# shiyuan0806/SVDFormer_PointSea

Measured on AMD Instinct MI355X. Metric: train-step samples/sec (PCN, B=32, 2048->16384 pts), higher is better.
Workload: dtype bf16; 1 GPU; SVDFormer PCN train step: render + fwd + get_loss + bwd + Adam; global_batch=32, per_gpu_batch=32, points_in=2048, points_out=16384, params=58092521, parallelism=single

## Files before the change

### include/pcops.h

```cpp
#ifndef PCOPS_H_
#define PCOPS_H_

#ifdef __cplusplus
extern "C" {
#endif

typedef struct ihipStream_t *pcops_stream_t;

enum pcops_status {
  PCOPS_OK = 0,
  PCOPS_ERR_INVALID = 1,
  PCOPS_ERR_LAUNCH = 2,
  PCOPS_ERR_WORKSPACE = 3,
  PCOPS_ERR_UNSUPPORTED = 4
};

const char *pcops_status_string(int status);
int pcops_abi_version(void);


unsigned long long pcops_fps_workspace_bytes(int B, int N);
int pcops_furthest_point_sampling(const float *xyz, int B, int N, int M, int *idx, void *workspace,
                                  unsigned long long workspace_bytes, pcops_stream_t stream);
int pcops_furthest_point_sampling_counts(const float *xyz, const int *counts, int B, int N, int M, int *idx,
// ... 200 lines not shown
int pcops_batchnorm_bwd(const void *dy, const void *y, const void *x, int dtype, long long rows, int C,
                        const float *gamma, const float *save_mean, const float *save_invstd, int batch_stats, int act,
                        float slope, void *dx, void *dres, float *dgamma, float *dbeta, void *workspace,
                        unsigned long long workspace_bytes, pcops_stream_t stream);
int pcops_batchnorm_fwd_save(const void *x, int dtype, const void *res, int res_dtype, long long rows, int C,
                             const float *gamma, const float *beta, float *running_mean, float *running_var,
                             float momentum, float eps, int batch_stats, int act, float slope, void *y,
                             float *save_mean, float *save_invstd, float *save_coef, unsigned char *save_mask,
                             void *workspace, unsigned long long workspace_bytes, long long *num_batches_tracked,
                             pcops_stream_t stream);
int pcops_batchnorm_bwd_saved(const void *dy, const float *save_coef, const unsigned char *save_mask, const void *x,
                              int dtype, long long rows, int C, const float *gamma, const float *save_mean,
                              const float *save_invstd, int batch_stats, int act, float slope, void *dx, void *dres,
                              float *dgamma, float *dbeta, void *workspace, unsigned long long workspace_bytes,
                              pcops_stream_t stream);

int pcops_conv3x3_fwd(const void *x, const void *w, int N, int H, int W, int C, void *y, pcops_stream_t stream);
int pcops_conv3x3_fwd_res(const void *x, const void *w, int N, int H, int W, int C, const void *res, void *y,
                          pcops_stream_t stream);
unsigned long long pcops_conv3x3_wgrad_workspace_bytes(int C);
int pcops_conv3x3_wgrad(const void *x, const void *dy, int N, int H, int W, int C, void *dw, int dw_dtype,
                        int dw_ohwi, void *workspace, unsigned long long workspace_bytes, pcops_stream_t stream);

int pcops_conv3x3_c1_fwd(const float *x, const float *w, int N, int H, int W, void *y, pcops_stream_t stream);
unsigned long long pcops_conv3x3_c1_wgrad_workspace_bytes(void);
int pcops_conv3x3_c1_wgrad(const float *x, const void *dy, int N, int H, int W, void *dw, int dw_dtype, void *workspace,
                           unsigned long long workspace_bytes, pcops_stream_t stream);

int pcops_pcsa_forward(const void *x, int x_dtype, const void *gates, int gates_dtype, const float *basis, int patches,
                       int K, int C, void *out, pcops_stream_t stream);
int pcops_pcsa_backward(const void *x, int x_dtype, const void *dout, int dout_dtype, const void *gates,
                        int gates_dtype, const float *basis, int patches, int K, int C, void *dx, void *dgates,
                        pcops_stream_t stream);

// ... 14 lines not shown
```

### svdformer_pointsea_amd/_lib.py

```python
import ctypes
import os
import threading

import torch

_HERE = os.path.dirname(os.path.abspath(__file__))
LIB_PATH = os.environ.get("PCOPS_LIB_PATH") or os.path.join(_HERE, "_lib", "libpcops.so")

_lib = None

P = ctypes.c_void_p
I = ctypes.c_int
F = ctypes.c_float
D = ctypes.c_double
LL = ctypes.c_longlong
ULL = ctypes.c_ulonglong

_SIGS = {
    "pcops_status_string": (ctypes.c_char_p, [I]),
    "pcops_abi_version": (I, []),
    "pcops_fps_workspace_bytes": (ULL, [I, I]),
    "pcops_furthest_point_sampling": (I, [P, I, I, I, P, P, ULL, P]),
    "pcops_furthest_point_sampling_counts": (I, [P, P, I, I, I, P, P, ULL, P]),
    "pcops_gather_points": (I, [P, P, I, I, I, I, P, P]),
# ... 53 lines not shown
    "pcops_layernorm_bwd_ex": (I, [P, I, LL, P, P, P, I, P, I, P, P, P, I, I, P, P, P, P, P, I, P, ULL, P]),
    "pcops_adam_flat": (I, [P, P, P, LL, LL, P, P, P, P, D, P, D, D, D, D, I, P]),
    "pcops_blend_fwd": (I, [P, I, P, P, LL, P, I, P]),
    "pcops_blend_bwd": (I, [P, I, P, I, P, P, LL, P, P, P, P]),
    "pcops_sum_rows": (I, [P, I, LL, P, I, P]),
    "pcops_wgrad_skinny_workspace_bytes": (ULL, [I, I]),
    "pcops_wgrad_skinny": (I, [P, P, LL, I, I, P, I, P, ULL, P]),
    "pcops_colsum_workspace_bytes": (ULL, [LL, I]),
    "pcops_colsum": (I, [P, I, LL, I, P, I, P, ULL, P]),
    "pcops_colsum_ld": (I, [P, I, LL, I, LL, P, I, P, ULL, P]),
    "pcops_batchnorm_workspace_bytes": (ULL, [LL, I]),
    "pcops_batchnorm_fwd": (I, [P, I, P, I, LL, I, P, P, P, P, F, F, I, I, F, P, P, P, P, ULL, P, P]),
    "pcops_batchnorm_bwd": (I, [P, P, P, I, LL, I, P, P, P, I, I, F, P, P, P, P, P, ULL, P]),
    "pcops_batchnorm_fwd_save": (I, [P, I, P, I, LL, I, P, P, P, P, F, F, I, I, F, P, P, P, P, P, P, ULL, P, P]),
    "pcops_batchnorm_bwd_saved": (I, [P, P, P, P, I, LL, I, P, P, P, I, I, F, P, P, P, P, P, ULL, P]),
    "pcops_conv3x3_fwd": (I, [P, P, I, I, I, I, P, P]),
    "pcops_conv3x3_fwd_res": (I, [P, P, I, I, I, I, P, P, P]),
    "pcops_conv3x3_wgrad_workspace_bytes": (ULL, [I]),
    "pcops_conv3x3_wgrad": (I, [P, P, I, I, I, I, P, I, I, P, ULL, P]),
    "pcops_conv3x3_c1_fwd": (I, [P, P, I, I, I, P, P]),
    "pcops_conv3x3_c1_wgrad_workspace_bytes": (ULL, []),
    "pcops_conv3x3_c1_wgrad": (I, [P, P, I, I, I, P, I, P, ULL, P]),
    "pcops_pcsa_forward": (I, [P, I, P, I, P, I, I, I, P, P]),
    "pcops_pcsa_backward": (I, [P, I, P, I, P, I, P, I, I, I, P, P, P]),
    "pcops_points2depth_workspace_bytes": (ULL, [I, I, I, I]),
    "pcops_points2depth": (I, [P, P, P, I, I, I, I, I, P, P, ULL, P]),
    "pcops_points2grid": (I, [P, P, P, P, I, I, I, I, I, P, P]),
    "pcops_grid2image_workspace_bytes": (ULL, [I, I, I]),
    "pcops_grid2image": (I, [P, P, I, I, I, P, P, ULL, P]),
}

# ... 278 lines not shown
```

### svdformer_pointsea_amd/batchnorm.py

```python
import os

import torch
from torch import nn

from ._lib import Workspace, call, lib, ptr, stream_of

_DT = {torch.float32: 0, torch.bfloat16: 1}
ACT_NONE, ACT_RELU, ACT_LEAKY = 0, 1, 2
ENABLED = os.environ.get("PCOPS_BN", "1") != "0"


def _rows_c(x):
    C = x.shape[1]
    return x.numel() // C, C


def _switch(name):
    return os.environ.get(name, "1") != "0"


def _mask_source(act, has_res):
    if act == ACT_NONE:
        return "y"
    if has_res:
        return "bits" if _switch("PCOPS_BN_MASK_BITS") else "y"
    return "coef" if _switch("PCOPS_BN_RECOMPUTE_MASK") else "y"


class _BNAct(torch.autograd.Function):
    @staticmethod
    def forward(ctx, x, res, weight, bias, rmean, rvar, nbt, batch_stats, momentum, eps, act, slope):
        rows, C = _rows_c(x)
        y = torch.empty_like(x)
        smean = torch.empty(C, dtype=torch.float32, device=x.device)
        sinv = torch.empty(C, dtype=torch.float32, device=x.device)
        src = _mask_source(act, res is not None)
        coef = mask = None
        with torch.cuda.device(x.device):
            nbytes = lib().pcops_batchnorm_workspace_bytes(rows, C)
            ws = Workspace.get(x.device, nbytes)
            if src == "y":
                call("batchnorm_fwd", lib().pcops_batchnorm_fwd, ptr(x), _DT[x.dtype], ptr(res),
                     _DT[res.dtype] if res is not None else 0, rows, C, ptr(weight), ptr(bias), ptr(rmean),
                     ptr(rvar), float(momentum), float(eps), int(batch_stats), act, float(slope), ptr(y), ptr(smean),
                     ptr(sinv), ptr(ws), nbytes, ptr(nbt), stream_of(x))
            else:
                coef = torch.empty(2 * C, dtype=torch.float32, device=x.device)
                if src == "bits":
                    mask = torch.empty(rows * C // 8, dtype=torch.uint8, device=x.device)
                call("batchnorm_fwd_save", lib().pcops_batchnorm_fwd_save, ptr(x), _DT[x.dtype], ptr(res),
                     _DT[res.dtype] if res is not None else 0, rows, C, ptr(weight), ptr(bias), ptr(rmean),
                     ptr(rvar), float(momentum), float(eps), int(batch_stats), act, float(slope), ptr(y), ptr(smean),
                     ptr(sinv), ptr(coef), ptr(mask), ptr(ws), nbytes, ptr(nbt), stream_of(x))
        ctx.save_for_backward(x, y if act != ACT_NONE and src == "y" else None, weight, smean, sinv,
                              coef if src == "coef" else None, mask)
        ctx.cfg = (batch_stats, act, slope, res is not None, src)
# ... 9 lines not shown
        dres = torch.empty_like(x) if has_res and ctx.needs_input_grad[1] else None
        need_w = weight is not None and ctx.needs_input_grad[2]
        dgamma = torch.empty(C, dtype=torch.float32, device=x.device) if need_w else None
        dbeta = torch.empty(C, dtype=torch.float32, device=x.device) if ctx.needs_input_grad[3] else None
        with torch.cuda.device(x.device):
            nbytes = lib().pcops_batchnorm_workspace_bytes(rows, C)
            ws = Workspace.get(x.device, nbytes)
            if src == "y":
                call("batchnorm_bwd", lib().pcops_batchnorm_bwd, ptr(gy), ptr(y), ptr(x), _DT[x.dtype], rows, C,
                     ptr(weight), ptr(smean), ptr(sinv), int(batch_stats), act, float(slope), ptr(dx), ptr(dres),
                     ptr(dgamma), ptr(dbeta), ptr(ws), nbytes, stream_of(x))
            else:
                call("batchnorm_bwd_saved", lib().pcops_batchnorm_bwd_saved, ptr(gy), ptr(coef), ptr(mask), ptr(x),
                     _DT[x.dtype], rows, C, ptr(weight), ptr(smean), ptr(sinv), int(batch_stats), act, float(slope),
                     ptr(dx), ptr(dres), ptr(dgamma), ptr(dbeta), ptr(ws), nbytes, stream_of(x))
        return dx, dres, dgamma, dbeta, None, None, None, None, None, None, None, None


def _fusable(x, bn, residual):
    if not (ENABLED and x.is_cuda and x.dim() == 4 and x.dtype in _DT and isinstance(bn, nn.BatchNorm2d)):
        return False
    C = x.shape[1]
    if C % 8 or C > 512 or x.numel() == 0 or not x.is_contiguous(memory_format=torch.channels_last):
        return False
    if bn.weight is None or bn.weight.dtype != torch.float32 or bn.momentum is None:
        return False
    if x.data_ptr() % 16:
        return False
    if residual is not None and (residual.shape != x.shape or residual.dtype not in _DT
                                 or not residual.is_contiguous(memory_format=torch.channels_last)
                                 or residual.data_ptr() % 16):
        return False
    return True


def _activation(out, act, slope):
    if act == ACT_RELU:
        return torch.relu(out)
    if act == ACT_LEAKY:
        return torch.nn.functional.leaky_relu(out, slope)
    return out


def bn_act(x, bn, act=ACT_NONE, slope=0.0, residual=None):
    if not _fusable(x, bn, residual):
        out = bn(x)
        if residual is not None:
            out = out + residual
        return _activation(out, act, slope)
    batch_stats = bn.training or bn.running_mean is None
    update = bn.training and bn.running_mean is not None
    rm = bn.running_mean if (update or not batch_stats) else None
    rv = bn.running_var if (update or not batch_stats) else None
    nbt = bn.num_batches_tracked if update else None
    return _BNAct.apply(x, residual, bn.weight, bn.bias, rm, rv, nbt, batch_stats, bn.momentum, bn.eps, act, slope)


def _act_of(m):
    if isinstance(m, nn.ReLU):
        return ACT_RELU, 0.0
    if isinstance(m, nn.LeakyReLU):
        return ACT_LEAKY, float(m.negative_slope)
    return None


def run_sequential(seq, x, conv_fn=None):
    mods = list(seq)
    i = 0
    while i < len(mods):
        m = mods[i]
# ... 14 lines not shown
```

### svdformer_pointsea_amd/conv.py

```python
import os

import torch
from torch import nn

from ._lib import Workspace, call, lib, ptr, stream_of

ENABLED = os.environ.get("PCOPS_CONV3X3", "1") != "0"
_CHANNELS = (16, 32)


def _ohwi(w):
    return w.to(torch.bfloat16).permute(0, 2, 3, 1).contiguous()


class _Conv3x3(torch.autograd.Function):
    @staticmethod
    def forward(ctx, x, w):
        N, C, H, W = x.shape
        y = torch.empty((N, C, H, W), dtype=torch.bfloat16, device=x.device, memory_format=torch.channels_last)
        with torch.cuda.device(x.device):
            call("conv3x3_fwd", lib().pcops_conv3x3_fwd, ptr(x), ptr(_ohwi(w)), N, H, W, C, ptr(y), stream_of(x))
        ctx.save_for_backward(x, w)
        return y

# ... 12 lines not shown
                gw = _Conv3x3._wgrad(x, w, gy)
        return gx, gw

    @staticmethod
    def _wgrad(x, w, gy):
        N, C, H, W = x.shape
        gw = torch.empty_like(w)
        ohwi = int(w.is_contiguous(memory_format=torch.channels_last) and not w.is_contiguous())
        if not (ohwi or w.is_contiguous()):
            gw = torch.empty(w.shape, dtype=w.dtype, device=w.device)
        nbytes = lib().pcops_conv3x3_wgrad_workspace_bytes(C)
        ws = Workspace.get(x.device, nbytes)
        call("conv3x3_wgrad", lib().pcops_conv3x3_wgrad, ptr(x), ptr(gy), N, H, W, C, ptr(gw),
             0 if w.dtype == torch.float32 else 1, ohwi, ptr(ws), nbytes, stream_of(x))
        return gw


class _Conv3x3Skip(torch.autograd.Function):

    @staticmethod
    def forward(ctx, x, w):
        ctx.set_materialize_grads(False)
        y = _Conv3x3.forward(ctx, x, w)
        return y, x.view_as(x)

    @staticmethod
    def backward(ctx, gy, gskip):
        x, w = ctx.saved_tensors
        N, C, H, W = x.shape
        gx = gw = None
# ... 4 lines not shown
            if ctx.needs_input_grad[0]:
                wt = w.to(torch.bfloat16).flip(2, 3).permute(1, 2, 3, 0).contiguous()
                gx = torch.empty_like(x)
                if gskip is None:
                    call("conv3x3_dgrad", lib().pcops_conv3x3_fwd, ptr(gy), ptr(wt), N, H, W, C, ptr(gx),
                         stream_of(x))
                else:
                    r = gskip.to(torch.bfloat16).contiguous(memory_format=torch.channels_last)
                    call("conv3x3_dgrad_res", lib().pcops_conv3x3_fwd_res, ptr(gy), ptr(wt), N, H, W, C, ptr(r),
                         ptr(gx), stream_of(x))
            if ctx.needs_input_grad[1]:
                gw = _Conv3x3._wgrad(x, w, gy)
        return gx, gw


class _Conv3x3C1(torch.autograd.Function):

    @staticmethod
    def forward(ctx, x, w):
        N, _, H, W = x.shape
        y = torch.empty((N, 16, H, W), dtype=torch.bfloat16, device=x.device, memory_format=torch.channels_last)
        with torch.cuda.device(x.device):
            call("conv3x3_c1_fwd", lib().pcops_conv3x3_c1_fwd, ptr(x), ptr(w.float().contiguous()), N, H, W, ptr(y),
                 stream_of(x))
        ctx.save_for_backward(x, w)
        return y

    @staticmethod
    def backward(ctx, gy):
        x, w = ctx.saved_tensors
# ... 22 lines not shown

def eligible(x, conv):
    if not (ENABLED and isinstance(conv, nn.Conv2d) and x.is_cuda and x.dim() == 4 and x.dtype == torch.bfloat16):
        return False
    C = x.shape[1]
    return (conv.kernel_size == (3, 3) and conv.stride == (1, 1) and conv.padding == (1, 1)
            and conv.dilation == (1, 1) and conv.groups == 1 and conv.bias is None and conv.padding_mode == "zeros"
            and C in _CHANNELS and conv.in_channels == C and conv.out_channels == C
            and conv.weight.dtype in (torch.float32, torch.bfloat16)
            and x.is_contiguous(memory_format=torch.channels_last) and x.data_ptr() % 16 == 0)


SKIP_FUSED = os.environ.get("PCOPS_CONV_SKIP", "1") != "0"


def conv3x3_skip(x, conv):
    w = conv.weight
    if SKIP_FUSED and eligible(x, conv) and w.dtype in (torch.float32, torch.bfloat16) and torch.is_grad_enabled():
        return _Conv3x3Skip.apply(x, w)
    return conv3x3(x, conv), x


def conv3x3(x, conv, weight=None):
    w = conv.weight if weight is None else weight
    if eligible(x, conv) and w.dtype in (torch.float32, torch.bfloat16):
        return _Conv3x3.apply(x, w)
    if stem_eligible(x, conv):
        return _Conv3x3C1.apply(x, w)
    return conv(x)
```

### svdformer_pointsea_amd/csrc/batchnorm.hip

```cpp
#include <atomic>
#include <cstdlib>

#include "common.h"

namespace {

struct V8 {
  float v[8];
};
typedef __bf16 bf16x8_t __attribute__((ext_vector_type(8)));

template <int DT>
__device__ __forceinline__ void ld8(V8 &o, const void *p, long long e) {
  if constexpr (DT == 0) {
    const float4 a = *reinterpret_cast<const float4 *>(reinterpret_cast<const float *>(p) + e);
    const float4 b = *reinterpret_cast<const float4 *>(reinterpret_cast<const float *>(p) + e + 4);
    o.v[0] = a.x, o.v[1] = a.y, o.v[2] = a.z, o.v[3] = a.w, o.v[4] = b.x, o.v[5] = b.y, o.v[6] = b.z, o.v[7] = b.w;
  } else {
    const bf16x8_t a = *reinterpret_cast<const bf16x8_t *>(reinterpret_cast<const __bf16 *>(p) + e);
#pragma unroll
    for (int k = 0; k < 8; ++k) o.v[k] = (float)a[k];
  }
}
template <int DT>
// ... 109 lines not shown
}

struct BnFin {
  const void *x;
  const float *gamma, *beta;
  float *rmean, *rvar;
  float momentum, eps;
  float *mean_io, *invstd_io, *dgamma, *dbeta;
  int eval;
  float *coef;
  long long *nbt;
  long long rows;
  int C;
};

template <int MODE, int DT>
__device__ __forceinline__ void bn_final_col(int c, double s0, double s1, const BnFin &f) {
  const int C = f.C;
  const double n = (double)f.rows;
  const double g = f.gamma ? (double)f.gamma[c] : 1.0;
  if constexpr (MODE == 0) {
    const double k = DT == 0 ? (double)reinterpret_cast<const float *>(f.x)[c]
                             : (double)(float)reinterpret_cast<const __bf16 *>(f.x)[c];
    const double m1 = s0 / n;
    double var = s1 / n - m1 * m1;
    if (var < 0.0) var = 0.0;
    const double mean = k + m1;
    const float invstd = 1.0f / sqrtf((float)var + f.eps);
    f.mean_io[c] = (float)mean;
    f.invstd_io[c] = invstd;
    if (f.rmean) {
      f.rmean[c] = (float)(f.momentum * mean + (1.0 - f.momentum) * (double)f.rmean[c]);
      const double unbiased = f.rows > 1 ? var * n / (n - 1.0) : var;
      f.rvar[c] = (float)(f.momentum * unbiased + (1.0 - f.momentum) * (double)f.rvar[c]);
    }
    if (f.nbt && c == 0) f.nbt[0] += 1;
    const double sc = g * (double)invstd;
    f.coef[c] = (float)sc;
    f.coef[C + c] = (float)((f.beta ? (double)f.beta[c] : 0.0) - (double)(float)mean * sc);
  } else {
    const double inv = (double)f.invstd_io[c];
    if (f.dgamma) f.dgamma[c] = (float)(s1 * inv);
    if (f.dbeta) f.dbeta[c] = (float)s0;
    const double ca = g * inv;
    double cb = 0.0, cc = 0.0;
    if (!f.eval) {
      cb = -g * inv * inv * inv * s1 / n;
      cc = -ca * s0 / n - cb * (double)f.mean_io[c];
    }
    f.coef[c] = (float)ca;
    f.coef[C + c] = (float)cb;
    f.coef[2 * C + c] = (float)cc;
  }
}
// ... 131 lines not shown
    for (int i = 0; i < 16; ++i) {
      a += (double)pa[i];
      b += (double)pb[i];
    }
  }
  red[0][grp][cl] = a;
  red[1][grp][cl] = b;
  __syncthreads();
  if (grp != 0 || c >= C) return;
  double s0 = 0.0, s1 = 0.0;
  for (int i = 0; i < 16; ++i) {
    s0 += red[0][i][cl];
    s1 += red[1][i][cl];
  }
  bn_final_col<MODE, DT>(c, s0, s1, fin);
}

__global__ void bn_eval_coef_kernel(int C, const float *__restrict__ gamma, const float *__restrict__ beta,
                                    const float *__restrict__ rmean, const float *__restrict__ rvar, float eps,
                                    float *__restrict__ mean_out, float *__restrict__ invstd_out,
                                    float *__restrict__ coef) {
  const int c = blockIdx.x * blockDim.x + threadIdx.x;
  if (c >= C) return;
  const float invstd = 1.0f / sqrtf(rvar[c] + eps);
  const float g = gamma ? gamma[c] : 1.f;
  const float sc = g * invstd;
  mean_out[c] = rmean[c];
  invstd_out[c] = invstd;
  coef[c] = sc;
  coef[C + c] = (beta ? beta[c] : 0.f) - rmean[c] * sc;
// ... 175 lines not shown

extern "C" unsigned long long pcops_batchnorm_workspace_bytes(long long rows, int C) {
  if (!bn_shape_ok(rows, C)) return 0;
  int chunks;
  long long rpc;
  bn_shape(rows, C, chunks, rpc);
  return ((unsigned long long)chunks * 2 * C + 3ULL * C) * sizeof(float);
}

namespace {

int bn_fwd(const void *x, int dtype, const void *res, int res_dtype, long long rows, int C, const float *gamma,
           const float *beta, float *running_mean, float *running_var, float momentum, float eps, int batch_stats,
           int act, float slope, void *y, float *save_mean, float *save_invstd, float *coef_out, unsigned char *mask,
           void *workspace, unsigned long long workspace_bytes, long long *num_batches_tracked,
           pcops_stream_t stream) {
  if (rows < 0 || C <= 0 || (dtype != 0 && dtype != 1) || act < 0 || act > 2) return PCOPS_ERR_INVALID;
  if (res && res_dtype != 0 && res_dtype != 1) return PCOPS_ERR_INVALID;
  if (rows == 0) return PCOPS_OK;
  if (!bn_shape_ok(rows, C)) return PCOPS_ERR_UNSUPPORTED;
  if (!x || !y || !save_mean || !save_invstd) return PCOPS_ERR_INVALID;
  if (!batch_stats && (!running_mean || !running_var)) return PCOPS_ERR_INVALID;
  if ((running_mean == nullptr) != (running_var == nullptr)) return PCOPS_ERR_INVALID;
  if (!workspace || workspace_bytes < pcops_batchnorm_workspace_bytes(rows, C)) return PCOPS_ERR_WORKSPACE;
  hipStream_t s = (hipStream_t)stream;
  int chunks;
  long long rpc;
  bn_shape(rows, C, chunks, rpc);
  float *part = (float *)workspace;
  float *coef = coef_out ? coef_out : part + (long long)chunks * 2 * C;
  if (batch_stats) {
    BnFin fin{x,         gamma,   beta,    running_mean, running_var, momentum,
              eps,       save_mean, save_invstd, nullptr, nullptr,     0,
              coef,      running_mean ? num_batches_tracked : nullptr, rows, C};
    if (dtype == 0)
      launch_stats<0>(0, kSrcY, x, nullptr, nullptr, nullptr, nullptr, rows, C, 0.f, part, chunks, rpc, fin, s);
    else
      launch_stats<1>(0, kSrcY, x, nullptr, nullptr, nullptr, nullptr, rows, C, 0.f, part, chunks, rpc, fin, s);
  } else {
    hipLaunchKernelGGL(bn_eval_coef_kernel, dim3((C + 255) / 256), dim3(256), 0, s, C, gamma, beta, running_mean,
                       running_var, eps, save_mean, save_invstd, coef);
  }
  const unsigned n8 = (unsigned)(rows * C / 8);
  const int rt = res ? res_dtype : -1;
  if (dtype == 0) {
    if (rt < 0) launch_apply<0, -1>(act, x, res, coef, C, n8, slope, y, mask, s);
    else if (rt == 0) launch_apply<0, 0>(act, x, res, coef, C, n8, slope, y, mask, s);
    else launch_apply<0, 1>(act, x, res, coef, C, n8, slope, y, mask, s);
  } else {
    if (rt < 0) launch_apply<1, -1>(act, x, res, coef, C, n8, slope, y, mask, s);
// ... 70 lines not shown
}

extern "C" int pcops_batchnorm_fwd_save(const void *x, int dtype, const void *res, int res_dtype, long long rows,
                                        int C, const float *gamma, const float *beta, float *running_mean,
                                        float *running_var, float momentum, float eps, int batch_stats, int act,
                                        float slope, void *y, float *save_mean, float *save_invstd, float *save_coef,
                                        unsigned char *save_mask, void *workspace,
                                        unsigned long long workspace_bytes, long long *num_batches_tracked,
                                        pcops_stream_t stream) {
  if (!save_coef) return PCOPS_ERR_INVALID;
  return bn_fwd(x, dtype, res, res_dtype, rows, C, gamma, beta, running_mean, running_var, momentum, eps, batch_stats,
                act, slope, y, save_mean, save_invstd, save_coef, save_mask, workspace, workspace_bytes,
                num_batches_tracked, stream);
}

extern "C" int pcops_batchnorm_bwd_saved(const void *dy, const float *save_coef, const unsigned char *save_mask,
                                         const void *x, int dtype, long long rows, int C, const float *gamma,
                                         const float *save_mean, const float *save_invstd, int batch_stats, int act,
                                         float slope, void *dx, void *dres, float *dgamma, float *dbeta,
                                         void *workspace, unsigned long long workspace_bytes, pcops_stream_t stream) {
  if (save_mask)
    return bn_bwd(kSrcBits, dy, save_mask, nullptr, x, dtype, rows, C, gamma, save_mean, save_invstd, batch_stats, act,
                  slope, dx, dres, dgamma, dbeta, workspace, workspace_bytes, stream);
  return bn_bwd(kSrcCoef, dy, nullptr, save_coef, x, dtype, rows, C, gamma, save_mean, save_invstd, batch_stats, act,
                slope, dx, dres, dgamma, dbeta, workspace, workspace_bytes, stream);
}
```

### svdformer_pointsea_amd/csrc/conv.hip

```cpp
#include "common.h"

namespace {

typedef __bf16 bf16x8 __attribute__((ext_vector_type(8)));
typedef __bf16 bf16x4 __attribute__((ext_vector_type(4)));
typedef short short4v __attribute__((ext_vector_type(4)));
typedef float f32x4 __attribute__((ext_vector_type(4)));

constexpr int kTH = 4;
constexpr int kTW = 64;
[[maybe_unused]] constexpr int kLW = kTW + 2;

__device__ __forceinline__ f32x4 mfma16(const bf16x8 &a, const bf16x8 &b, const f32x4 &c) {
  return __builtin_amdgcn_mfma_f32_16x16x32_bf16(a, b, c, 0, 0, 0);
}

template <int C, int R, int L, int NTH = 256>
struct Stage {
  static constexpr int VPP = C / 8, TOT = R * L * VPP, PER = (TOT + NTH - 1) / NTH;
  bf16x8 v[PER];
  __device__ __forceinline__ void load(const __bf16 *__restrict__ x, int n, int hb, int wb, int H, int W) {
#pragma unroll
    for (int j = 0; j < PER; ++j) {
      const int i = threadIdx.x + NTH * j;
// ... 68 lines not shown
      __bf16 *yp = y + e0;
      bf16x4 rv[MT];
      if (res)
#pragma unroll
        for (int mt = 0; mt < MT; ++mt) rv[mt] = *reinterpret_cast<const bf16x4 *>(res + e0 + 16 * mt);
#pragma unroll
      for (int mt = 0; mt < MT; ++mt) {
        bf16x4 o;
#pragma unroll
        for (int r = 0; r < 4; ++r) o[r] = (__bf16)acc[mt][r];
        if (res)
#pragma unroll
          for (int r = 0; r < 4; ++r) o[r] = (__bf16)((float)o[r] + (float)rv[mt][r]);
        *reinterpret_cast<bf16x4 *>(yp + 16 * mt) = o;
      }
    }
  }
}

template <int CI, int CO>
__global__ __launch_bounds__(256) void conv3x3_wgrad_kernel(const __bf16 *__restrict__ x,
                                                            const __bf16 *__restrict__ dy, int N, int H, int W,
                                                            float *__restrict__ part) {
#if defined(__HIP_DEVICE_COMPILE__)
  constexpr int MT = CO / 16, NT = CI / 16;
  constexpr int kXT = (kTH + 2) * kLW * CI, kGT = kTH * kTW * CO, kE = 9 * CO * CI;
  constexpr int kBytes = (2 * (kXT + kGT) > 4 * kE ? 2 * (kXT + kGT) : 4 * kE);
  __shared__ float4 arena[(kBytes + 15) / 16];
  __bf16 *xt = reinterpret_cast<__bf16 *>(arena);
  __bf16 *gt = xt + kXT;
// ... 298 lines not shown
#pragma unroll
  for (int i = 0; i < kC1Out * 9; ++i) {
    float v = acc[i];
#pragma unroll
    for (int off = 32; off >= 1; off >>= 1) v += __shfl_xor(v, off, 64);
    if (lane == 0) red[wv][i] = v;
  }
  __syncthreads();
  for (int i = threadIdx.x; i < kC1Out * 9; i += 256)
    part[(long long)blockIdx.x * kC1Out * 9 + i] = ((red[0][i] + red[1][i]) + red[2][i]) + red[3][i];
}

}

namespace {
int conv3x3_fwd_impl(const void *x, const void *w, int N, int H, int W, int C, const void *res, void *y,
                     pcops_stream_t stream) {
  if (N < 0 || H < 0 || W < 0) return PCOPS_ERR_INVALID;
  if (N == 0 || H == 0 || W == 0) return PCOPS_OK;
  if (!conv_ok(N, H, W, C)) return PCOPS_ERR_UNSUPPORTED;
  if (!x || !w || !y) return PCOPS_ERR_INVALID;
  const __bf16 *rp = (const __bf16 *)res;
  hipStream_t s = (hipStream_t)stream;
  const bool wide = W % 112 == 0;
  const int TW = wide ? 112 : 64;
  const long long tiles = (long long)((W + TW - 1) / TW) * ((H + kTH - 1) / kTH) * N;
  const dim3 grid((unsigned)(((tiles + 7) / 8) * 8));
  const __bf16 *xp = (const __bf16 *)x, *wp = (const __bf16 *)w;
  __bf16 *yp = (__bf16 *)y;
  if (C == 16) {
    if (wide) hipLaunchKernelGGL((conv3x3_fwd_kernel<16, 16, 112>), grid, dim3(256), 0, s, xp, wp, yp, H, W, N, rp);
    else hipLaunchKernelGGL((conv3x3_fwd_kernel<16, 16, 64>), grid, dim3(256), 0, s, xp, wp, yp, H, W, N, rp);
  } else {
    if (wide) hipLaunchKernelGGL((conv3x3_fwd_kernel<32, 32, 112>), grid, dim3(256), 0, s, xp, wp, yp, H, W, N, rp);
    else hipLaunchKernelGGL((conv3x3_fwd_kernel<32, 32, 64>), grid, dim3(256), 0, s, xp, wp, yp, H, W, N, rp);
  }
  PC_CHECK_LAUNCH();
  return PCOPS_OK;
}
}

extern "C" int pcops_conv3x3_fwd(const void *x, const void *w, int N, int H, int W, int C, void *y,
                                 pcops_stream_t stream) {
  return conv3x3_fwd_impl(x, w, N, H, W, C, nullptr, y, stream);
}

extern "C" int pcops_conv3x3_fwd_res(const void *x, const void *w, int N, int H, int W, int C, const void *res,
                                     void *y, pcops_stream_t stream) {
  if (!res) return PCOPS_ERR_INVALID;
  return conv3x3_fwd_impl(x, w, N, H, W, C, res, y, stream);
}

extern "C" unsigned long long pcops_conv3x3_wgrad_workspace_bytes(int C) {
  if (C != 16 && C != 32) return 0;
  return (unsigned long long)(wgrad_blocks(C) + kSplit) * 9 * C * C * sizeof(float);
}

extern "C" int pcops_conv3x3_wgrad(const void *x, const void *dy, int N, int H, int W, int C, void *dw, int dw_dtype,
                                   int dw_ohwi, void *workspace, unsigned long long workspace_bytes,
                                   pcops_stream_t stream) {
  if (N < 0 || H < 0 || W < 0 || !dw || (dw_dtype != 0 && dw_dtype != 1)) return PCOPS_ERR_INVALID;
  hipStream_t s = (hipStream_t)stream;
  if (N == 0 || H == 0 || W == 0) {
    if (pc_memset_async(dw, 0, (dw_dtype == 0 ? 4 : 2) * 9 * C * C, s) != hipSuccess) return PCOPS_ERR_LAUNCH;
    return PCOPS_OK;
// ... 59 lines not shown
```

### svdformer_pointsea_amd/svdformer.py

```python
import numpy as np
import torch
import torch.nn.functional as F
from torch import nn

from .attention import (PosEmbedding, SDG_Decoder, block_sum, block_sum_cat, cross_attention, linear, linear_skinny,
                        self_attention, to_channels, to_tokens)
from .chamfer3D import chamfer_3DDist
from .model_utils import (SharedFPS, edge_features, fps_subsample, group_local, sample_and_group_knn,
                          sample_and_group_knn_cl)
from ._lib import fork
from .batchnorm import ACT_RELU, bn_act, run_sequential
from .conv import conv3x3, conv3x3_skip
from .pointnet2_utils import furthest_point_sample, gather_operation


def _lin(conv, x):
    return linear(x, conv.weight.view(conv.weight.shape[0], -1), conv.bias)


class _MaxK(torch.autograd.Function):

    @staticmethod
    def forward(ctx, x):
        from ._lib import call, lib, ptr, stream_of

        B, S, K, C = x.shape
        out = torch.empty(B, S, C, dtype=x.dtype, device=x.device)
# ... 298 lines not shown

class BasicBlock(nn.Module):
    expansion = 1

    def __init__(self, inplanes, planes, stride=1, downsample=None):
        super().__init__()
        self.conv1 = nn.Conv2d(inplanes, planes, 3, stride=stride, padding=1, bias=False)
        self.bn1 = nn.BatchNorm2d(planes)
        self.relu = nn.ReLU(inplace=True)
        self.conv2 = nn.Conv2d(planes, planes, 3, padding=1, bias=False)
        self.bn2 = nn.BatchNorm2d(planes)
        self.downsample = downsample

    def forward(self, x):
        if self.downsample is None:
            y1, identity = conv3x3_skip(x, self.conv1)
        else:
            identity = run_sequential(self.downsample, x)
            y1 = conv3x3(x, self.conv1)
        out = bn_act(y1, self.bn1, ACT_RELU)
        return bn_act(conv3x3(out, self.conv2), self.bn2, ACT_RELU, residual=identity)


def _resnet_layers(feature_size=16, layers=(2, 2, 2, 2)):
    inplanes = feature_size
    out = []
    for i, n in enumerate(layers):
        planes = feature_size * (2 ** i)
        stride = 1 if i == 0 else 2
        down = None
        if stride != 1 or inplanes != planes:
            down = nn.Sequential(nn.Conv2d(inplanes, planes, 1, stride=stride, bias=False), nn.BatchNorm2d(planes))
        blocks = [BasicBlock(inplanes, planes, stride, down)]
        inplanes = planes
        blocks += [BasicBlock(inplanes, planes) for _ in range(1, n)]
        out.append(nn.Sequential(*blocks))
# ... 245 lines not shown
```

Before: 702.1 samples/s.

## Fuse BatchNorm batch statistics into the 3x3 conv forward epilogue

The 3x3 conv forward now has a persistent-loop variant that computes per-channel count, mean and M2 partials in its epilogue while writing the output. It emits one stats row per block. A new BN entry point reduces these partials with a Chan-style combine instead of re-reading the conv output to compute batch statistics. The ResNet BasicBlocks use this path during training. It removes a full read pass over each conv activation. The risks are that stats come from bf16-rounded outputs and that the persistent grid may schedule differently from the original per-tile conv kernel.

New measurement: 702.1 samples/s. Within noise of the previous version (-0.0%).

```diff
diff --git a/include/pcops.h b/include/pcops.h
--- a/include/pcops.h
+++ b/include/pcops.h
@@ -238,10 +238,19 @@
                               const float *save_invstd, int batch_stats, int act, float slope, void *dx, void *dres,
                               float *dgamma, float *dbeta, void *workspace, unsigned long long workspace_bytes,
                               pcops_stream_t stream);
+int pcops_batchnorm_fwd_from_stats(const void *x, int dtype, const void *res, int res_dtype, long long rows, int C,
+                                   const float *gamma, const float *beta, float *running_mean, float *running_var,
+                                   float momentum, float eps, int batch_stats, int act, float slope, void *y,
+                                   float *save_mean, float *save_invstd, float *save_coef, unsigned char *save_mask,
+                                   void *workspace, unsigned long long workspace_bytes, long long *num_batches_tracked,
+                                   const void *stats, int stats_rows, pcops_stream_t stream);
 
 int pcops_conv3x3_fwd(const void *x, const void *w, int N, int H, int W, int C, void *y, pcops_stream_t stream);
 int pcops_conv3x3_fwd_res(const void *x, const void *w, int N, int H, int W, int C, const void *res, void *y,
                           pcops_stream_t stream);
+unsigned long long pcops_conv3x3_fwd_stats_workspace_bytes(int N, int H, int W, int C);
+int pcops_conv3x3_fwd_stats(const void *x, const void *w, int N, int H, int W, int C, void *y, void *stats,
+                            unsigned long long stats_bytes, pcops_stream_t stream);
 unsigned long long pcops_conv3x3_wgrad_workspace_bytes(int C);
 int pcops_conv3x3_wgrad(const void *x, const void *dy, int N, int H, int W, int C, void *dw, int dw_dtype,
                         int dw_ohwi, void *workspace, unsigned long long workspace_bytes, pcops_stream_t stream);
diff --git a/svdformer_pointsea_amd/_lib.py b/svdformer_pointsea_amd/_lib.py
--- a/svdformer_pointsea_amd/_lib.py
+++ b/svdformer_pointsea_amd/_lib.py
@@ -91,7 +91,10 @@
     "pcops_batchnorm_bwd": (I, [P, P, P, I, LL, I, P, P, P, I, I, F, P, P, P, P, P, ULL, P]),
     "pcops_batchnorm_fwd_save": (I, [P, I, P, I, LL, I, P, P, P, P, F, F, I, I, F, P, P, P, P, P, P, ULL, P, P]),
     "pcops_batchnorm_bwd_saved": (I, [P, P, P, P, I, LL, I, P, P, P, I, I, F, P, P, P, P, P, ULL, P]),
+    "pcops_batchnorm_fwd_from_stats": (I, [P, I, P, I, LL, I, P, P, P, P, F, F, I, I, F, P, P, P, P, P, P, ULL, P, P, I, P]),
     "pcops_conv3x3_fwd": (I, [P, P, I, I, I, I, P, P]),
+    "pcops_conv3x3_fwd_stats_workspace_bytes": (ULL, [I, I, I, I]),
+    "pcops_conv3x3_fwd_stats": (I, [P, P, I, I, I, I, P, P, ULL, P]),
     "pcops_conv3x3_fwd_res": (I, [P, P, I, I, I, I, P, P, P]),
     "pcops_conv3x3_wgrad_workspace_bytes": (ULL, [I]),
     "pcops_conv3x3_wgrad": (I, [P, P, I, I, I, I, P, I, I, P, ULL, P]),
diff --git a/svdformer_pointsea_amd/batchnorm.py b/svdformer_pointsea_amd/batchnorm.py
--- a/svdformer_pointsea_amd/batchnorm.py
+++ b/svdformer_pointsea_amd/batchnorm.py
@@ -29,7 +29,7 @@
 
 class _BNAct(torch.autograd.Function):
     @staticmethod
-    def forward(ctx, x, res, weight, bias, rmean, rvar, nbt, batch_stats, momentum, eps, act, slope):
+    def forward(ctx, x, res, weight, bias, rmean, rvar, nbt, batch_stats, momentum, eps, act, slope, stats=None):
         rows, C = _rows_c(x)
         y = torch.empty_like(x)
         smean = torch.empty(C, dtype=torch.float32, device=x.device)
@@ -39,7 +39,15 @@
         with torch.cuda.device(x.device):
             nbytes = lib().pcops_batchnorm_workspace_bytes(rows, C)
             ws = Workspace.get(x.device, nbytes)
-            if src == "y":
+            if stats is not None:
+                coef = torch.empty(2 * C, dtype=torch.float32, device=x.device)
+                if src == "bits":
+                    mask = torch.empty(rows * C // 8, dtype=torch.uint8, device=x.device)
+                call("batchnorm_fwd", lib().pcops_batchnorm_fwd_from_stats, ptr(x), _DT[x.dtype], ptr(res),
+                     _DT[res.dtype] if res is not None else 0, rows, C, ptr(weight), ptr(bias), ptr(rmean),
+                     ptr(rvar), float(momentum), float(eps), 1, act, float(slope), ptr(y), ptr(smean), ptr(sinv),
+                     ptr(coef), ptr(mask), ptr(ws), nbytes, ptr(nbt), ptr(stats), stats.shape[0], stream_of(x))
+            elif src == "y":
                 call("batchnorm_fwd", lib().pcops_batchnorm_fwd, ptr(x), _DT[x.dtype], ptr(res),
                      _DT[res.dtype] if res is not None else 0, rows, C, ptr(weight), ptr(bias), ptr(rmean),
                      ptr(rvar), float(momentum), float(eps), int(batch_stats), act, float(slope), ptr(y), ptr(smean),
@@ -79,7 +87,7 @@
                 call("batchnorm_bwd_saved", lib().pcops_batchnorm_bwd_saved, ptr(gy), ptr(coef), ptr(mask), ptr(x),
                      _DT[x.dtype], rows, C, ptr(weight), ptr(smean), ptr(sinv), int(batch_stats), act, float(slope),
                      ptr(dx), ptr(dres), ptr(dgamma), ptr(dbeta), ptr(ws), nbytes, stream_of(x))
-        return dx, dres, dgamma, dbeta, None, None, None, None, None, None, None, None
+        return dx, dres, dgamma, dbeta, None, None, None, None, None, None, None, None, None
 
 
 def _fusable(x, bn, residual):
@@ -107,7 +115,7 @@
     return out
 
 
-def bn_act(x, bn, act=ACT_NONE, slope=0.0, residual=None):
+def bn_act(x, bn, act=ACT_NONE, slope=0.0, residual=None, stats=None):
     if not _fusable(x, bn, residual):
         out = bn(x)
         if residual is not None:
@@ -118,7 +126,11 @@
     rm = bn.running_mean if (update or not batch_stats) else None
     rv = bn.running_var if (update or not batch_stats) else None
     nbt = bn.num_batches_tracked if update else None
-    return _BNAct.apply(x, residual, bn.weight, bn.bias, rm, rv, nbt, batch_stats, bn.momentum, bn.eps, act, slope)
+    if not (update and x.dtype == torch.bfloat16 and stats is not None and stats.dtype == torch.float32
+            and stats.dim() == 3 and stats.shape[1:] == (3, x.shape[1]) and stats.is_contiguous()):
+        stats = None
+    return _BNAct.apply(x, residual, bn.weight, bn.bias, rm, rv, nbt, batch_stats, bn.momentum, bn.eps, act, slope,
+                        stats)
 
 
 def _act_of(m):
diff --git a/svdformer_pointsea_amd/conv.py b/svdformer_pointsea_amd/conv.py
--- a/svdformer_pointsea_amd/conv.py
+++ b/svdformer_pointsea_amd/conv.py
@@ -50,6 +50,34 @@
         call("conv3x3_wgrad", lib().pcops_conv3x3_wgrad, ptr(x), ptr(gy), N, H, W, C, ptr(gw),
              0 if w.dtype == torch.float32 else 1, ohwi, ptr(ws), nbytes, stream_of(x))
         return gw
+
+
+def _fwd_stats(x, w):
+    N, C, H, W = x.shape
+    y = torch.empty((N, C, H, W), dtype=torch.bfloat16, device=x.device, memory_format=torch.channels_last)
+    with torch.cuda.device(x.device):
+        nbytes = lib().pcops_conv3x3_fwd_stats_workspace_bytes(N, H, W, C)
+        stats = torch.empty((nbytes // (12 * C), 3, C), dtype=torch.float32, device=x.device)
+        call("conv3x3_fwd", lib().pcops_conv3x3_fwd_stats, ptr(x), ptr(_ohwi(w)), N, H, W, C, ptr(y), ptr(stats),
+             nbytes, stream_of(x))
+    return y, stats
+
+
+class _Conv3x3Stats(torch.autograd.Function):
+
+    @staticmethod
+    def forward(ctx, x, w):
+        ctx.set_materialize_grads(False)
+        y, stats = _fwd_stats(x, w)
+        ctx.save_for_backward(x, w)
+        ctx.mark_non_differentiable(stats)
+        return y, stats
+
+    @staticmethod
+    def backward(ctx, gy, _gstats):
+        if gy is None:
+            return None, None
+        return _Conv3x3.backward(ctx, gy)
 
 
 class _Conv3x3Skip(torch.autograd.Function):
@@ -84,6 +112,21 @@
         return gx, gw
 
 
+class _Conv3x3SkipStats(torch.autograd.Function):
+
+    @staticmethod
+    def forward(ctx, x, w):
+        ctx.set_materialize_grads(False)
+        y, stats = _fwd_stats(x, w)
+        ctx.save_for_backward(x, w)
+        ctx.mark_non_differentiable(stats)
+        return y, x.view_as(x), stats
+
+    @staticmethod
+    def backward(ctx, gy, gskip, _gstats):
+        return _Conv3x3Skip.backward(ctx, gy, gskip)
+
+
 class _Conv3x3C1(torch.autograd.Function):
 
     @staticmethod
@@ -136,11 +179,35 @@
 SKIP_FUSED = os.environ.get("PCOPS_CONV_SKIP", "1") != "0"
 
 
-def conv3x3_skip(x, conv):
+def stats_enabled():
+    return os.environ.get("PCOPS_CONV_BN_STATS", "1") != "0"
+
+
+def _bn_takes_stats(bn):
+    return (stats_enabled() and torch.is_grad_enabled() and isinstance(bn, nn.BatchNorm2d) and bn.training
+            and bn.running_mean is not None)
+
+
+def conv3x3_skip(x, conv, bn=None):
     w = conv.weight
-    if SKIP_FUSED and eligible(x, conv) and w.dtype in (torch.float32, torch.bfloat16) and torch.is_grad_enabled():
+    ok = eligible(x, conv) and w.dtype in (torch.float32, torch.bfloat16)
+    if bn is not None:
+        if ok and _bn_takes_stats(bn):
+            if SKIP_FUSED:
+                return _Conv3x3SkipStats.apply(x, w)
+            y, stats = _Conv3x3Stats.apply(x, w)
+            return y, x, stats
+        return (*conv3x3_skip(x, conv), None)
+    if SKIP_FUSED and ok and torch.is_grad_enabled():
         return _Conv3x3Skip.apply(x, w)
     return conv3x3(x, conv), x
+
+
+def conv3x3_stats(x, conv, bn):
+    w = conv.weight
+    if eligible(x, conv) and w.dtype in (torch.float32, torch.bfloat16) and _bn_takes_stats(bn):
+        return _Conv3x3Stats.apply(x, w)
+    return conv3x3(x, conv), None
 
 
 def conv3x3(x, conv, weight=None):
diff --git a/svdformer_pointsea_amd/csrc/batchnorm.hip b/svdformer_pointsea_amd/csrc/batchnorm.hip
--- a/svdformer_pointsea_amd/csrc/batchnorm.hip
+++ b/svdformer_pointsea_amd/csrc/batchnorm.hip
@@ -147,6 +147,24 @@
   int C;
 };
 
+__device__ __forceinline__ void bn_fwd_finish(int c, double mean, double var, const BnFin &f) {
+  const int C = f.C;
+  const double n = (double)f.rows;
+  const double g = f.gamma ? (double)f.gamma[c] : 1.0;
+  const float invstd = 1.0f / sqrtf((float)var + f.eps);
+  f.mean_io[c] = (float)mean;
+  f.invstd_io[c] = invstd;
+  if (f.rmean) {
+    f.rmean[c] = (float)(f.momentum * mean + (1.0 - f.momentum) * (double)f.rmean[c]);
+    const double unbiased = f.rows > 1 ? var * n / (n - 1.0) : var;
+    f.rvar[c] = (float)(f.momentum * unbiased + (1.0 - f.momentum) * (double)f.rvar[c]);
+  }
+  if (f.nbt && c == 0) f.nbt[0] += 1;
+  const double sc = g * (double)invstd;
+  f.coef[c] = (float)sc;
+  f.coef[C + c] = (float)((f.beta ? (double)f.beta[c] : 0.0) - (double)(float)mean * sc);
+}
+
 template <int MODE, int DT>
 __device__ __forceinline__ void bn_final_col(int c, double s0, double s1, const BnFin &f) {
   const int C = f.C;
@@ -158,19 +176,7 @@
     const double m1 = s0 / n;
     double var = s1 / n - m1 * m1;
     if (var < 0.0) var = 0.0;
-    const double mean = k + m1;
-    const float invstd = 1.0f / sqrtf((float)var + f.eps);
-    f.mean_io[c] = (float)mean;
-    f.invstd_io[c] = invstd;
-    if (f.rmean) {
-      f.rmean[c] = (float)(f.momentum * mean + (1.0 - f.momentum) * (double)f.rmean[c]);
-      const double unbiased = f.rows > 1 ? var * n / (n - 1.0) : var;
-      f.rvar[c] = (float)(f.momentum * unbiased + (1.0 - f.momentum) * (double)f.rvar[c]);
-    }
-    if (f.nbt && c == 0) f.nbt[0] += 1;
-    const double sc = g * (double)invstd;
-    f.coef[c] = (float)sc;
-    f.coef[C + c] = (float)((f.beta ? (double)f.beta[c] : 0.0) - (double)(float)mean * sc);
+    bn_fwd_finish(c, k + m1, var, f);
   } else {
     const double inv = (double)f.invstd_io[c];
     if (f.dgamma) f.dgamma[c] = (float)(s1 * inv);
@@ -332,6 +338,61 @@
     s1 += red[1][i][cl];
   }
   bn_final_col<MODE, DT>(c, s0, s1, fin);
+}
+
+constexpr int kFsThreads = 1024, kFsGroups = kFsThreads / 8, kFsRows = 16;
+
+__global__ __launch_bounds__(kFsThreads) void bn_from_stats_kernel(const float *__restrict__ stats, int srows,
+                                                                   BnFin fin) {
+  __shared__ double red[3][kFsGroups][8];
+  __shared__ double red2[3][8][8];
+  const int C = fin.C;
+  const int cl = threadIdx.x & 7, grp = threadIdx.x >> 3;
+  const int c = blockIdx.x * 8 + cl;
+  const double k = (double)stats[C + c];
+  double n = 0.0, s1 = 0.0, s2 = 0.0;
+  for (int r0 = grp; r0 < srows; r0 += kFsGroups * kFsRows) {
+    float ni[kFsRows], mi[kFsRows], qi[kFsRows];
+#pragma unroll
+    for (int j = 0; j < kFsRows; ++j) {
+      const int r = r0 + j * kFsGroups;
+      const float *row = stats + (long long)(r < srows ? r : 0) * 3 * C + c;
+      ni[j] = r < srows ? row[0] : 0.f;
+      mi[j] = row[C];
+      qi[j] = r < srows ? row[2 * C] : 0.f;
+    }
+#pragma unroll
+    for (int j = 0; j < kFsRows; ++j) {
+      const double d = (double)mi[j] - k;
+      n += (double)ni[j];
+      s1 += (double)ni[j] * d;
+      s2 += (double)qi[j] + (double)ni[j] * (d * d);
+    }
+  }
+  red[0][grp][cl] = n;
+  red[1][grp][cl] = s1;
+  red[2][grp][cl] = s2;
+  __syncthreads();
+  if (threadIdx.x < 3 * 64) {
+    const int h = threadIdx.x >> 6, g8 = (threadIdx.x >> 3) & 7;
+    double v = 0.0;
+#pragma unroll
+    for (int i = 0; i < kFsGroups / 8; ++i) v += red[h][g8 * (kFsGroups / 8) + i][cl];
+    red2[h][g8][cl] = v;
+  }
+  __syncthreads();
+  if (threadIdx.x >= 8) return;
+  n = s1 = s2 = 0.0;
+#pragma unroll
+  for (int i = 0; i < 8; ++i) {
+    n += red2[0][i][cl];
+    s1 += red2[1][i][cl];
+    s2 += red2[2][i][cl];
+  }
+  const double m1 = n > 0.0 ? s1 / n : 0.0;
+  double var = n > 0.0 ? (s2 - s1 * m1) / n : 0.0;
+  if (var < 0.0) var = 0.0;
+  bn_fwd_finish(c, k + m1, var, fin);
 }
 
 __global__ void bn_eval_coef_kernel(int C, const float *__restrict__ gamma, const float *__restrict__ beta,
@@ -537,9 +598,10 @@
            const float *beta, float *running_mean, float *running_var, float momentum, float eps, int batch_stats,
            int act, float slope, void *y, float *save_mean, float *save_invstd, float *coef_out, unsigned char *mask,
            void *workspace, unsigned long long workspace_bytes, long long *num_batches_tracked,
-           pcops_stream_t stream) {
+           pcops_stream_t stream, const float *stats = nullptr, int stats_rows = 0) {
   if (rows < 0 || C <= 0 || (dtype != 0 && dtype != 1) || act < 0 || act > 2) return PCOPS_ERR_INVALID;
   if (res && res_dtype != 0 && res_dtype != 1) return PCOPS_ERR_INVALID;
+  if (stats && (!batch_stats || stats_rows <= 0 || ((unsigned long long)stats & 3))) return PCOPS_ERR_INVALID;
   if (rows == 0) return PCOPS_OK;
   if (!bn_shape_ok(rows, C)) return PCOPS_ERR_UNSUPPORTED;
   if (!x || !y || !save_mean || !save_invstd) return PCOPS_ERR_INVALID;
@@ -556,7 +618,9 @@
     BnFin fin{x,         gamma,   beta,    running_mean, running_var, momentum,
               eps,       save_mean, save_invstd, nullptr, nullptr,     0,
               coef,      running_mean ? num_batches_tracked : nullptr, rows, C};
-    if (dtype == 0)
+    if (stats)
+      hipLaunchKernelGGL(bn_from_stats_kernel, dim3(C / 8), dim3(kFsThreads), 0, s, stats, stats_rows, fin);
+    else if (dtype == 0)
       launch_stats<0>(0, kSrcY, x, nullptr, nullptr, nullptr, nullptr, rows, C, 0.f, part, chunks, rpc, fin, s);
     else
       launch_stats<1>(0, kSrcY, x, nullptr, nullptr, nullptr, nullptr, rows, C, 0.f, part, chunks, rpc, fin, s);
@@ -657,6 +721,19 @@
                 num_batches_tracked, stream);
 }
 
+extern "C" int pcops_batchnorm_fwd_from_stats(const void *x, int dtype, const void *res, int res_dtype, long long rows,
+                                              int C, const float *gamma, const float *beta, float *running_mean,
+                                              float *running_var, float momentum, float eps, int batch_stats,
+                                              int act, float slope, void *y, float *save_mean, float *save_invstd,
+                                              float *save_coef, unsigned char *save_mask, void *workspace,
+                                              unsigned long long workspace_bytes, long long *num_batches_tracked,
+                                              const void *stats, int stats_rows, pcops_stream_t stream) {
+  if (!save_coef || !stats || !batch_stats) return PCOPS_ERR_INVALID;
+  return bn_fwd(x, dtype, res, res_dtype, rows, C, gamma, beta, running_mean, running_var, momentum, eps, batch_stats,
+                act, slope, y, save_mean, save_invstd, save_coef, save_mask, workspace, workspace_bytes,
+                num_batches_tracked, stream, (const float *)stats, stats_rows);
+}
+
 extern "C" int pcops_batchnorm_bwd_saved(const void *dy, const float *save_coef, const unsigned char *save_mask,
                                          const void *x, int dtype, long long rows, int C, const float *gamma,
                                          const float *save_mean, const float *save_invstd, int batch_stats, int act,
diff --git a/svdformer_pointsea_amd/csrc/conv.hip b/svdformer_pointsea_amd/csrc/conv.hip
--- a/svdformer_pointsea_amd/csrc/conv.hip
+++ b/svdformer_pointsea_amd/csrc/conv.hip
@@ -1,3 +1,5 @@
+#include <cstdlib>
+
 #include "common.h"
 
 namespace {
@@ -106,6 +108,153 @@
           for (int r = 0; r < 4; ++r) o[r] = (__bf16)((float)o[r] + (float)rv[mt][r]);
         *reinterpret_cast<bf16x4 *>(yp + 16 * mt) = o;
       }
+    }
+  }
+}
+
+#ifndef PCOPS_CONV_LOOP_WAVES32
+#define PCOPS_CONV_LOOP_WAVES32 2
+#endif
+template <int CI, int CO, int TW, bool STATS>
+__global__ __launch_bounds__(256, CI == 32 ? PCOPS_CONV_LOOP_WAVES32 : 4) void conv3x3_fwd_loop_kernel(const __bf16 *__restrict__ x,
+                                                               const __bf16 *__restrict__ w, __bf16 *__restrict__ y,
+                                                               int H, int W, int N, const __bf16 *__restrict__ res,
+                                                               int parts, float *__restrict__ stats) {
+  constexpr int KC = (9 * CI + 31) / 32;
+  constexpr int MT = CO / 16;
+  constexpr int LW = TW + 2;
+  constexpr int NTU = CI == 32 ? 1 : TW / 16;
+  __shared__ __attribute__((aligned(16))) __bf16 tile[(kTH + 2) * LW * CI];
+  const int tw = (W + TW - 1) / TW, th = (H + kTH - 1) / kTH;
+  const long long tiles = (long long)N * th * tw;
+  const int l = threadIdx.x & 63, wv = threadIdx.x >> 6, g = l >> 4, i16 = l & 15;
+  bf16x8 a[MT][KC];
+#pragma unroll
+  for (int c = 0; c < KC; ++c) {
+    const int k0 = 32 * c + 8 * g, tap = k0 / CI, ci0 = k0 % CI;
+#pragma unroll
+    for (int mt = 0; mt < MT; ++mt)
+      a[mt][c] = tap < 9 ? *reinterpret_cast<const bf16x8 *>(w + ((16 * mt + i16) * 9 + tap) * CI + ci0) : bf16x8{};
+  }
+  Stage<CI, kTH + 2, LW> st;
+  auto fetch = [&](long long t) {
+    st.load(x, (int)(t / ((long long)th * tw)), (int)((t / tw) % th) * kTH - 1, (int)(t % tw) * TW - 1, H, W);
+  };
+  const long long per = (tiles + parts - 1) / parts, lo = (blockIdx.x % parts) * per, hi = min(tiles, lo + per);
+  const long long t0 = lo + blockIdx.x / parts, ts = gridDim.x / parts;
+  float sk[MT][4], s0[MT][4], s1[MT][4], cnt = 0.f;
+#pragma unroll
+  for (int mt = 0; mt < MT; ++mt)
+#pragma unroll
+    for (int r = 0; r < 4; ++r) sk[mt][r] = s0[mt][r] = s1[mt][r] = 0.f;
+  if (t0 < hi) fetch(t0);
+  for (long long t = t0; t < hi; t += ts) {
+    __syncthreads();
+    st.store(tile);
+    __syncthreads();
+    if (t + ts < hi) fetch(t + ts);
+    const int n = (int)(t / ((long long)th * tw)), h0 = (int)((t / tw) % th) * kTH, w0 = (int)(t % tw) * TW;
+    const int orow = h0 + wv;
+#pragma unroll NTU
+    for (int nt = 0; nt < TW / 16; ++nt) {
+      f32x4 acc[MT];
+#pragma unroll
+      for (int mt = 0; mt < MT; ++mt) acc[mt] = f32x4{0.f, 0.f, 0.f, 0.f};
+      const int pc = 16 * nt + i16;
+#pragma unroll
+      for (int c = 0; c < KC; ++c) {
+        const int k0 = 32 * c + 8 * g;
+        const int tap = k0 / CI < 9 ? k0 / CI : 8;
+        const int ci0 = k0 % CI, dh = tap / 3, dw = tap % 3;
+        const bf16x8 b = *reinterpret_cast<const bf16x8 *>(tile + ((wv + dh) * LW + pc + dw) * CI + ci0);
+#pragma unroll
+        for (int mt = 0; mt < MT; ++mt) acc[mt] = mfma16(a[mt][c], b, acc[mt]);
+      }
+      const int ow = w0 + pc;
+      if (orow < H && ow < W) {
+        const long long e0 = (((long long)n * H + orow) * W + ow) * CO + 4 * g;
+        __bf16 *yp = y + e0;
+        bf16x4 rv[MT];
+        if (res)
+#pragma unroll
+          for (int mt = 0; mt < MT; ++mt) rv[mt] = *reinterpret_cast<const bf16x4 *>(res + e0 + 16 * mt);
+        const bool first = cnt == 0.f;
+#pragma unroll
+        for (int mt = 0; mt < MT; ++mt) {
+          bf16x4 o;
+#pragma unroll
+          for (int r = 0; r < 4; ++r) o[r] = (__bf16)acc[mt][r];
+          if constexpr (STATS) {
+#pragma unroll
+            for (int r = 0; r < 4; ++r) {
+              const float v = (float)o[r];
+              sk[mt][r] = first ? v : sk[mt][r];
+              const float d = v - sk[mt][r];
+              s0[mt][r] += d;
+              s1[mt][r] = __builtin_fmaf(d, d, s1[mt][r]);
+            }
+          }
+          if (res)
+#pragma unroll
+            for (int r = 0; r < 4; ++r) o[r] = (__bf16)((float)o[r] + (float)rv[mt][r]);
+          *reinterpret_cast<bf16x4 *>(yp + 16 * mt) = o;
+        }
+        cnt += 1.f;
+      }
+    }
+  }
+  if constexpr (STATS) {
+    __shared__ double smean[4][CO], sm2[4][CO], scnt[4];
+    double nn = (double)cnt, mean[MT][4], m2[MT][4];
+#pragma unroll
+    for (int mt = 0; mt < MT; ++mt)
+#pragma unroll
+      for (int r = 0; r < 4; ++r) {
+        const double m = nn > 0.0 ? (double)s0[mt][r] / nn : 0.0;
+        const double q = (double)s1[mt][r] - (double)s0[mt][r] * m;
+        mean[mt][r] = nn > 0.0 ? (double)sk[mt][r] + m : 0.0;
+        m2[mt][r] = q > 0.0 ? q : 0.0;
+      }
+#pragma unroll
+    for (int off = 1; off < 16; off <<= 1) {
+      const double nb = __shfl_xor(nn, off, 64), nab = nn + nb;
+      const double fb = nab > 0.0 ? nb / nab : 0.0;
+#pragma unroll
+      for (int mt = 0; mt < MT; ++mt)
+#pragma unroll
+        for (int r = 0; r < 4; ++r) {
+          const double d = __shfl_xor(mean[mt][r], off, 64) - mean[mt][r];
+          m2[mt][r] = (m2[mt][r] + __shfl_xor(m2[mt][r], off, 64)) + d * d * (nn * fb);
+          mean[mt][r] = mean[mt][r] + d * fb;
+        }
+      nn = nab;
+    }
+    if (i16 == 0) {
+#pragma unroll
+      for (int mt = 0; mt < MT; ++mt)
+#pragma unroll
+        for (int r = 0; r < 4; ++r) {
+          smean[wv][16 * mt + 4 * g + r] = mean[mt][r];
+          sm2[wv][16 * mt + 4 * g + r] = m2[mt][r];
+        }
+      if (l == 0) scnt[wv] = nn;
+    }
+    __syncthreads();
+    if (threadIdx.x < CO) {
+      const int c = threadIdx.x;
+      double na = scnt[0], ma = smean[0][c], qa = sm2[0][c];
+#pragma unroll
+      for (int s = 1; s < 4; ++s) {
+        const double nb = scnt[s], nab = na + nb, fb = nab > 0.0 ? nb / nab : 0.0;
+        const double d = smean[s][c] - ma;
+        qa = (qa + sm2[s][c]) + d * d * (na * fb);
+        ma = ma + d * fb;
+        na = nab;
+      }
+      float *row = stats + (long long)blockIdx.x * 3 * CO;
+      row[c] = (float)na;
+      row[CO + c] = (float)ma;
+      row[2 * CO + c] = (float)qa;
     }
   }
 }
@@ -434,6 +583,51 @@
 }
 
 namespace {
+constexpr int kFwdMaxBlocks = 4096;
+
+long long conv_fwd_tiles(int N, int H, int W) {
+  const int TW = W % 112 == 0 ? 112 : 64;
+  return (long long)((W + TW - 1) / TW) * ((H + kTH - 1) / kTH) * N;
+}
+
+int conv_fwd_loop_blocks(long long tiles, int C) {
+  if (const char *e = getenv("PCOPS_CONV_FWD_BLOCKS")) {
+    const int g = atoi(e);
+    if (g > 0) return g < 8 ? g : (g > kFwdMaxBlocks ? kFwdMaxBlocks : (g + 7) / 8 * 8);
+  }
+  const long long full = 256 * (C <= 16 ? 4 * 2 : PCOPS_CONV_LOOP_WAVES32), one = (tiles + 7) / 8 * 8;
+  return (int)(one < full ? one : full);
+}
+
+bool conv_fwd_loop() {
+  const char *e = getenv("PCOPS_CONV_FWD_LOOP");
+  return e && atoi(e) != 0;
+}
+
+template <bool STATS>
+void launch_fwd_loop(const __bf16 *xp, const __bf16 *wp, __bf16 *yp, int N, int H, int W, int C, const __bf16 *rp,
+                     float *stats, hipStream_t s) {
+  const bool wide = W % 112 == 0;
+  const int G = conv_fwd_loop_blocks(conv_fwd_tiles(N, H, W), C);
+  const dim3 grid(G);
+  const int parts = G < 8 ? G : 8;
+  if (C == 16) {
+    if (wide)
+      hipLaunchKernelGGL((conv3x3_fwd_loop_kernel<16, 16, 112, STATS>), grid, dim3(256), 0, s, xp, wp, yp, H, W, N, rp,
+                         parts, stats);
+    else
+      hipLaunchKernelGGL((conv3x3_fwd_loop_kernel<16, 16, 64, STATS>), grid, dim3(256), 0, s, xp, wp, yp, H, W, N, rp,
+                         parts, stats);
+  } else {
+    if (wide)
+      hipLaunchKernelGGL((conv3x3_fwd_loop_kernel<32, 32, 112, STATS>), grid, dim3(256), 0, s, xp, wp, yp, H, W, N, rp,
+                         parts, stats);
+    else
+      hipLaunchKernelGGL((conv3x3_fwd_loop_kernel<32, 32, 64, STATS>), grid, dim3(256), 0, s, xp, wp, yp, H, W, N, rp,
+                         parts, stats);
+  }
+}
+
 int conv3x3_fwd_impl(const void *x, const void *w, int N, int H, int W, int C, const void *res, void *y,
                      pcops_stream_t stream) {
   if (N < 0 || H < 0 || W < 0) return PCOPS_ERR_INVALID;
@@ -443,11 +637,15 @@
   const __bf16 *rp = (const __bf16 *)res;
   hipStream_t s = (hipStream_t)stream;
   const bool wide = W % 112 == 0;
-  const int TW = wide ? 112 : 64;
-  const long long tiles = (long long)((W + TW - 1) / TW) * ((H + kTH - 1) / kTH) * N;
+  const long long tiles = conv_fwd_tiles(N, H, W);
   const dim3 grid((unsigned)(((tiles + 7) / 8) * 8));
   const __bf16 *xp = (const __bf16 *)x, *wp = (const __bf16 *)w;
   __bf16 *yp = (__bf16 *)y;
+  if (conv_fwd_loop()) {
+    launch_fwd_loop<false>(xp, wp, yp, N, H, W, C, rp, nullptr, s);
+    PC_CHECK_LAUNCH();
+    return PCOPS_OK;
+  }
   if (C == 16) {
     if (wide) hipLaunchKernelGGL((conv3x3_fwd_kernel<16, 16, 112>), grid, dim3(256), 0, s, xp, wp, yp, H, W, N, rp);
     else hipLaunchKernelGGL((conv3x3_fwd_kernel<16, 16, 64>), grid, dim3(256), 0, s, xp, wp, yp, H, W, N, rp);
@@ -469,6 +667,25 @@
                                      void *y, pcops_stream_t stream) {
   if (!res) return PCOPS_ERR_INVALID;
   return conv3x3_fwd_impl(x, w, N, H, W, C, res, y, stream);
+}
+
+extern "C" unsigned long long pcops_conv3x3_fwd_stats_workspace_bytes(int N, int H, int W, int C) {
+  if (N <= 0 || H <= 0 || W <= 0 || !conv_ok(N, H, W, C)) return 0;
+  return (unsigned long long)conv_fwd_loop_blocks(conv_fwd_tiles(N, H, W), C) * 3 * C * sizeof(float);
+}
+
+extern "C" int pcops_conv3x3_fwd_stats(const void *x, const void *w, int N, int H, int W, int C, void *y, void *stats,
+                                       unsigned long long stats_bytes, pcops_stream_t stream) {
+  if (N < 0 || H < 0 || W < 0) return PCOPS_ERR_INVALID;
+  if (N == 0 || H == 0 || W == 0) return PCOPS_OK;
+  if (!conv_ok(N, H, W, C)) return PCOPS_ERR_UNSUPPORTED;
+  if (!x || !w || !y) return PCOPS_ERR_INVALID;
+  if (!stats || ((unsigned long long)stats & 3) || stats_bytes < pcops_conv3x3_fwd_stats_workspace_bytes(N, H, W, C))
+    return PCOPS_ERR_WORKSPACE;
+  launch_fwd_loop<true>((const __bf16 *)x, (const __bf16 *)w, (__bf16 *)y, N, H, W, C, nullptr, (float *)stats,
+                        (hipStream_t)stream);
+  PC_CHECK_LAUNCH();
+  return PCOPS_OK;
 }
 
 extern "C" unsigned long long pcops_conv3x3_wgrad_workspace_bytes(int C) {
diff --git a/svdformer_pointsea_amd/svdformer.py b/svdformer_pointsea_amd/svdformer.py
--- a/svdformer_pointsea_amd/svdformer.py
+++ b/svdformer_pointsea_amd/svdformer.py
@@ -10,7 +10,7 @@
                           sample_and_group_knn_cl)
 from ._lib import fork
 from .batchnorm import ACT_RELU, bn_act, run_sequential
-from .conv import conv3x3, conv3x3_skip
+from .conv import conv3x3, conv3x3_skip, conv3x3_stats
 from .pointnet2_utils import furthest_point_sample, gather_operation
 
 
@@ -339,12 +339,13 @@
 
     def forward(self, x):
         if self.downsample is None:
-            y1, identity = conv3x3_skip(x, self.conv1)
+            y1, identity, st1 = conv3x3_skip(x, self.conv1, self.bn1)
         else:
             identity = run_sequential(self.downsample, x)
-            y1 = conv3x3(x, self.conv1)
-        out = bn_act(y1, self.bn1, ACT_RELU)
-        return bn_act(conv3x3(out, self.conv2), self.bn2, ACT_RELU, residual=identity)
+            y1, st1 = conv3x3_stats(x, self.conv1, self.bn1)
+        out = bn_act(y1, self.bn1, ACT_RELU, stats=st1)
+        y2, st2 = conv3x3_stats(out, self.conv2, self.bn2)
+        return bn_act(y2, self.bn2, ACT_RELU, residual=identity, stats=st2)
 
 
 def _resnet_layers(feature_size=16, layers=(2, 2, 2, 2)):
```
